# Pixie8888/R3DFSSeg

Hardware: AMD Instinct MI355X
Metric: episodes/sec S3DIS 2-way 5-shot 2048-pt (MPTI+attention, train step: forward+backward+grad all-reduce+Adam) (higher is better)
Workload: dtype f32 (index-free GEMMs -- self-attention, 1x1 convolutions, weight gradients, the EdgeConv backward's edge GEMMs -- as bf16x3 split products on the bf16 MFMA with fp32 accumulate; every index-deciding result: fp32)

## Files before the change

### r3dfsseg_amd/csrc/edge_tile.h

```cpp
#pragma once
#include "common.h"

#define E2_PTS 4
#define E2_LD 68

static __device__ __forceinline__ f32x4 mfma16(float a, float b, f32x4 c) {
  return __builtin_amdgcn_mfma_f32_16x16x4f32(a, b, c, 0, 0, 0);
}

template <int RT>
static __device__ __forceinline__ void e2_rowgemm(const float* __restrict__ A, const float (&Bf)[16], int n, int g,
                                                  f32x4 (&acc)[RT]) {
#pragma unroll
  for (int t = 0; t < RT; ++t) acc[t] = f32x4{0.f, 0.f, 0.f, 0.f};
#pragma unroll
  for (int qk = 0; qk < 4; ++qk) {
    float4 av[RT];
#pragma unroll
    for (int t = 0; t < RT; ++t) av[t] = *(const float4*)(A + (16 * t + n) * E2_LD + 16 * g + 4 * qk);
#pragma unroll
    for (int s = 0; s < 4; ++s) {
#pragma unroll
      for (int t = 0; t < RT; ++t) {
        const float a = s == 0 ? av[t].x : s == 1 ? av[t].y : s == 2 ? av[t].z : av[t].w;
        acc[t] = mfma16(a, Bf[4 * qk + s], acc[t]);
      }
    }
  }
}

template <typename KernelT>
static int e2_resident_blocks(KernelT kernel, size_t lds, int cap) {
  if (hipFuncSetAttribute((const void*)kernel, hipFuncAttributeMaxDynamicSharedMemorySize, (int)lds) != hipSuccess) return 0;
  int per_cu = 0, dev = 0;
  hipDeviceProp_t prop;
  if (hipOccupancyMaxActiveBlocksPerMultiprocessor(&per_cu, kernel, 256, lds) != hipSuccess || hipGetDevice(&dev) != hipSuccess ||
      hipGetDeviceProperties(&prop, dev) != hipSuccess || per_cu <= 0)
    return 0;
  const int r = per_cu * prop.multiProcessorCount;
  return r < cap ? r : cap;
// ... 2 lines not shown
```

### r3dfsseg_amd/csrc/edgeconv.hip

```cpp
#include "edge_tile.h"

template <int RT>
__global__ __launch_bounds__(256) void r3d_edgeconv_kernel(
    const float* __restrict__ PQ, const int* __restrict__ idx, const float* __restrict__ W2,
    const float* __restrict__ s2, const float* __restrict__ t2, float* __restrict__ out, long ldo,
    int N, long total_points, int* __restrict__ argmax_out) {
  constexpr int K = 4 * RT, R = 16 * RT;
  extern __shared__ __attribute__((aligned(16))) float smem[];
  float* H = smem;
  float* Z = smem + R * E2_LD;
  const int tid = threadIdx.x, lane = tid & 63, w = tid >> 6;
  const int n = lane & 15, g = lane >> 4;
  const int c = 16 * w + n;
  float Bz[16];
#pragma unroll
  for (int s = 0; s < 16; ++s) Bz[s] = W2[c * 64 + 16 * g + s];
  const float s2c = s2[c], t2c = t2[c];
  const long units = total_points / E2_PTS;
  for (long item = blockIdx.x; item < units; item += gridDim.x) {
    const long u = r3d_xcd_swizzle((int)item, (int)units);
    const long pt0 = u * E2_PTS;
    const long cloud0 = (pt0 / N) * N;
    {
      const int my_idx = min(max(idx[(pt0 + w) * K + min(lane, K - 1)], 0), N - 1);
      const float q = PQ[(pt0 + w) * 128 + 64 + lane];
      float pv[K];
#pragma unroll
      for (int t = 0; t < K; ++t) pv[t] = PQ[(cloud0 + __builtin_amdgcn_readlane(my_idx, t)) * 128 + lane];
      float* hrow = H + (K * w) * E2_LD + lane;
#pragma unroll
      for (int t = 0; t < K; ++t) {
        const float h = pv[t] + q;
        hrow[t * E2_LD] = h > 0.f ? h : 0.2f * h;
      }
    }
    __syncthreads();
    f32x4 acc[RT];
    e2_rowgemm<RT>(H, Bz, n, g, acc);
#pragma unroll
    for (int t = 0; t < RT; ++t) {
#pragma unroll
      for (int i = 0; i < 4; ++i) {
        const float v = s2c * acc[t][i] + t2c;
        Z[(16 * t + 4 * g + i) * E2_LD + c] = v > 0.f ? v : 0.2f * v;
      }
    }
    __syncthreads();
    {
      const float* zp = Z + (K * w) * E2_LD + lane;
      float m = zp[0];
      int am = 0;
#pragma unroll
      for (int t = 1; t < K; ++t) {
        const float v = zp[t * E2_LD];
        if (v > m) { m = v; am = t; }
      }
      out[(pt0 + w) * ldo + lane] = m;
      if (argmax_out) argmax_out[(pt0 + w) * 64 + lane] = am;
    }
  }
}

template <int RT>
static int edgeconv_launch_rt(const float* PQ, const int32_t* idx, const float* W2, const float* s2, const float* t2, float* out,
                              long ldo, int N, long total_points, int32_t* argmax_out, hipStream_t st) {
  const size_t lds = sizeof(float) * ((size_t)2 * 16 * RT * E2_LD);
  static int resident = 0;
  if (!resident) {
    resident = e2_resident_blocks(r3d_edgeconv_kernel<RT>, lds, 1024);
    R3D_REQUIRE(resident > 0, "r3d_edgeconv_fwd: cannot reserve %zu B of LDS", lds);
  }
  const long units = total_points / E2_PTS;
  const int grid = (int)(units <= resident ? units : (resident & ~7));
  hipLaunchKernelGGL(r3d_edgeconv_kernel<RT>, dim3(grid), dim3(256), lds, st, PQ, idx, W2, s2, t2, out, ldo, N, total_points,
                     argmax_out);
  return R3D_OK;
}

extern "C" int r3d_edgeconv_fwd(const float* PQ, const int32_t* idx, const float* W2, const float* s2,
                                const float* t2, float* out, long ldo, int B, int N, int K,
                                int32_t* argmax_out, void* stream) {
  R3D_REQUIRE(PQ && idx && W2 && s2 && t2 && out, "r3d_edgeconv_fwd: null pointer");
  R3D_REQUIRE(B > 0 && N > 0 && ldo >= 64, "r3d_edgeconv_fwd: bad shape");
  R3D_REQUIRE(N % E2_PTS == 0, "r3d_edgeconv_fwd: N=%d must be a multiple of %d", N, E2_PTS);
  R3D_REQUIRE(K >= 4 && K <= 32 && K % 4 == 0, "r3d_edgeconv_fwd: K=%d unsupported (need K %% 4 == 0, 4..32)", K);
  hipStream_t st = (hipStream_t)stream;
  int rc = R3D_ERR_ARG;
#define E2_CASE(RT) \
  case RT: rc = edgeconv_launch_rt<RT>(PQ, idx, W2, s2, t2, out, ldo, N, (long)B * N, argmax_out, st); break
  switch (K / 4) {
    E2_CASE(1); E2_CASE(2); E2_CASE(3); E2_CASE(4); E2_CASE(5); E2_CASE(6); E2_CASE(7); E2_CASE(8);
  }
#undef E2_CASE
  if (rc) return rc;
  R3D_LAUNCH_CHECK("r3d_edgeconv_fwd");
  return R3D_OK;
}
```

### r3dfsseg_amd/csrc/edgeconv_train.hip

```cpp
#include <stdlib.h>
#include "edge_tile.h"

#define ET_LD 65
#define ET_MAXBLK 1024
#define EC_CHUNK 32

static __device__ __forceinline__ float lrelu(float v) { return v > 0.f ? v : 0.2f * v; }

struct EcGeom {
  int N, cpc;
  __host__ __device__ static EcGeom make(int N) { return EcGeom{N, (N + EC_CHUNK - 1) / EC_CHUNK}; }
  __device__ void range(int chunk, int& cloud, int& p0, int& p1) const {
    cloud = __builtin_amdgcn_readfirstlane(chunk / cpc);
    p0 = __builtin_amdgcn_readfirstlane(cloud * N + (chunk - cloud * cpc) * EC_CHUNK);
    p1 = __builtin_amdgcn_readfirstlane(min(p0 + EC_CHUNK, (cloud + 1) * N));
  }
};
static __device__ __forceinline__ int ec_seg(const r3d_segmap& cs, int cloud) {
  return __builtin_amdgcn_readfirstlane(cs.seg_of_row32(cloud));
}

template <int RT>
__global__ __launch_bounds__(256) void r3d_edge_stats1_kernel(const float* __restrict__ PQ, const int* __restrict__ idx,
                                                              EcGeom gm, int n_chunks, float* __restrict__ part,
// ... 200 lines not shown
        float bs = 0.f, es = 0.f;
#pragma unroll
        for (int t = 0; t < K; ++t) {
          const float v = grow[t * E2_LD];
          drow[t * 64] = v;
          bs += v;
          es += eh[t];
          sdye += v * eh[t];
        }
        sdy += bs;
        BE[(pt0 + w) * 128 + lane] = bs;
        BE[(pt0 + w) * 128 + 64 + lane] = es;
      }
    }
    float (*ps)[2][64] = (float (*)[2][64])dsm;
    ps[w][0][lane] = sdy;
    ps[w][1][lane] = sdye;
    __syncthreads();
    if (tid < 128) {
      const int v = tid >> 6, cc = tid & 63;
      part_bn[((long)chunk * 2 + v) * 64 + cc] = ((ps[0][v][cc] + ps[1][v][cc]) + ps[2][v][cc]) + ps[3][v][cc];
    }
    __syncthreads();
  }
  int tid2 = threadIdx.x;
  asm volatile("" : "+v"(tid2));
  const int w2 = tid2 >> 6, n2 = tid2 & 15, g2 = (tid2 >> 4) & 3;
  float* mypart = part_dw + (long)blockIdx.x * 4096;
#pragma unroll
  for (int i = 0; i < 4; ++i)
    *(float4*)(mypart + (16 * w2 + 4 * g2 + i) * 64 + 4 * n2) = float4{dw[0][i], dw[1][i], dw[2][i], dw[3][i]};
}

template <int RT>
__global__ __launch_bounds__(256) void r3d_edgeconv_train_fwd2_kernel(
    const float* __restrict__ PQ, const int* __restrict__ idx, const float* __restrict__ s1, const float* __restrict__ t1,
    long bn_stride, const float* __restrict__ W2, EcGeom gm, r3d_segmap cs , int n_chunks,
    int* __restrict__ argmax_out, float* __restrict__ zmax_out, float* __restrict__ zmin_out, int* __restrict__ argmin_out,
    float* __restrict__ part ) {
  constexpr int K = 4 * RT, R = 16 * RT;
  extern __shared__ __attribute__((aligned(16))) float smem[];
  float* H = smem;
  float* Z = smem + R * E2_LD;
  const int tid = threadIdx.x, lane = tid & 63, w = tid >> 6;
  const int n = lane & 15, g = lane >> 4;
  const int c = 16 * w + n;
  const int N = gm.N;
  float Bz[16];
#pragma unroll
  for (int s = 0; s < 16; ++s) Bz[s] = W2[c * 64 + 16 * g + s];
  for (int item = blockIdx.x; item < n_chunks; item += gridDim.x) {
    const int chunk = r3d_xcd_swizzle(item, n_chunks);
    int cloud, p0, p1;
    gm.range(chunk, cloud, p0, p1);
    const long cloud0 = (long)cloud * N;
    const long bo = (long)ec_seg(cs, cloud) * bn_stride;
    const float sc1 = s1[bo + lane], sh1 = t1[bo + lane];
    float za = 0.f, zb = 0.f;
    for (int pt0_ = p0; pt0_ < p1; pt0_ += E2_PTS) {
      const long pt0 = pt0_;
      {
        const int my_idx = min(max(idx[(pt0 + w) * K + min(lane, K - 1)], 0), N - 1);
        const float q = PQ[(pt0 + w) * 128 + 64 + lane];
        float pv[K];
#pragma unroll
        for (int t = 0; t < K; ++t) pv[t] = PQ[(cloud0 + __builtin_amdgcn_readlane(my_idx, t)) * 128 + lane];
        float* hrow = H + (K * w) * E2_LD + lane;
#pragma unroll
        for (int t = 0; t < K; ++t) hrow[t * E2_LD] = lrelu(sc1 * (pv[t] + q) + sh1);
      }
      __syncthreads();
      f32x4 acc[RT];
      e2_rowgemm<RT>(H, Bz, n, g, acc);
#pragma unroll
      for (int t = 0; t < RT; ++t) {
#pragma unroll
        for (int i = 0; i < 4; ++i) {
          const float z = acc[t][i];
          za += z;
          zb += z * z;
          Z[(16 * t + 4 * g + i) * E2_LD + c] = z;
        }
      }
      __syncthreads();
      {
        const float* zp = Z + (K * w) * E2_LD + lane;
        float zx = zp[0], zn = zx;
        int ax = 0, an = 0;
#pragma unroll
        for (int t = 1; t < K; ++t) {
          const float z = zp[t * E2_LD];
          if (z > zx) { zx = z; ax = t; }
          if (z < zn) { zn = z; an = t; }
        }
        const long o = (pt0 + w) * 64 + lane;
        zmax_out[o] = zx;
        zmin_out[o] = zn;
        argmax_out[o] = ax;
        argmin_out[o] = an;
      }
    }
    za += __shfl_xor(za, 16); zb += __shfl_xor(zb, 16);
    za += __shfl_xor(za, 32); zb += __shfl_xor(zb, 32);
    if (g == 0) {
      part[((long)chunk * 2 + 0) * 64 + c] = za;
      part[((long)chunk * 2 + 1) * 64 + c] = zb;
    }
  }
}

#define RV_RANGE 256
#define RV_CAP 12288
__global__ __launch_bounds__(1024) void r3d_edge_reverse_kernel(const int* __restrict__ idx, int N, int K, int n_clouds,
                                                                int* __restrict__ rev_ptr, int* __restrict__ rev) {
  __shared__ int cnt[RV_RANGE];
  __shared__ int off[RV_RANGE + 1];
  __shared__ int cur[RV_RANGE];
  __shared__ int buf[RV_CAP];
  __shared__ int wsum[16];
  __shared__ int below_s, b_s;
  const int tid = threadIdx.x, lane = tid & 63, w = tid >> 6;
  const int cloud = blockIdx.y;
  const int r0 = blockIdx.x * RV_RANGE, nr = min(RV_RANGE, N - r0);
  const long E = (long)N * K, gbase = (long)cloud * E;
  const int* lst = idx + gbase;
  if (tid < RV_RANGE) cnt[tid] = 0;
  if (tid == 0) below_s = 0;
  __syncthreads();
  int my_below = 0;
  for (long e0 = tid; e0 < E; e0 += 8 * 1024) {
    int jv[8];
#pragma unroll
    for (int u = 0; u < 8; ++u) jv[u] = lst[min(e0 + 1024 * u, E - 1)];
// ... 239 lines not shown

extern "C" long r3d_edgeconv_train_ws_words(int B, int N) { return (long)ET_MAXBLK * 4096 + (long)et_chunks(B, N) * 128 + 64; }

static void et_reduce_chunks(const float* part, int N, int clouds_a, int clouds_b, int n_seg, float* out, hipStream_t st) {
  const int cpc = EcGeom::make(N).cpc;
  hipLaunchKernelGGL(r3d_part_reduce_kernel, dim3(128 / 64, n_seg), dim3(1024), 0, st, part, clouds_a * cpc, clouds_b * cpc, 128,
                     out, 128L, 128, (float*)nullptr, 0L);
}

extern "C" int r3d_edge_stats1(const float* PQ, const int32_t* idx, int B, int N, int K, int clouds_a, int clouds_b,
                               float* sums_out, float* esum, float* ws, void* stream) {
  R3D_REQUIRE(PQ && idx && sums_out && ws, "r3d_edge_stats1: null pointer");
  int rc = et_check("r3d_edge_stats1", B, N, K, clouds_a, clouds_b);
  if (rc) return rc;
  hipStream_t st = (hipStream_t)stream;
  const EcGeom gm = EcGeom::make(N);
  const int n_chunks = et_chunks(B, N);
  const int grid = et_grid8(n_chunks, 2048);
#define E2_CASE(RT) \
  case RT: hipLaunchKernelGGL(r3d_edge_stats1_kernel<RT>, dim3(grid), dim3(256), 0, st, PQ, idx, gm, n_chunks, ws, esum); break
  switch (K / 4) {
    E2_CASE(1); E2_CASE(2); E2_CASE(3); E2_CASE(4); E2_CASE(5); E2_CASE(6); E2_CASE(7); E2_CASE(8);
  }
#undef E2_CASE
  et_reduce_chunks(ws, N, clouds_a, clouds_b, r3d_segmap{clouds_a, clouds_b}.n_seg(B), sums_out, st);
  R3D_LAUNCH_CHECK("r3d_edge_stats1");
  return R3D_OK;
}

template <int RT>
static int fwd2_launch_rt(int n_chunks, hipStream_t st, const float* PQ, const int32_t* idx, const float* s1, const float* t1,
                          long bn_stride, const float* W2, EcGeom gm, r3d_segmap cs, int32_t* argmax, float* zmax, float* zmin,
                          int32_t* argmin, float* ws) {
  const size_t lds = sizeof(float) * ((size_t)2 * 16 * RT * E2_LD);
  static int resident = 0;
  if (!resident) {
    resident = e2_resident_blocks(r3d_edgeconv_train_fwd2_kernel<RT>, lds, ET_MAXBLK);
    R3D_REQUIRE(resident > 0, "r3d_edgeconv_train_fwd_minmax: cannot reserve %zu B of LDS", lds);
  }
  const int grid = et_grid8(n_chunks, resident);
  hipLaunchKernelGGL(r3d_edgeconv_train_fwd2_kernel<RT>, dim3(grid), dim3(256), lds, st, PQ, idx, s1, t1, bn_stride, W2, gm, cs,
                     n_chunks, argmax, zmax, zmin, argmin, ws);
  return R3D_OK;
}

extern "C" int r3d_edgeconv_train_fwd_minmax(const float* PQ, const int32_t* idx, const float* s1, const float* t1,
                                             long bn_stride, const float* W2, int B, int N, int K, int clouds_a, int clouds_b,
                                             float* zmax, float* zmin, int32_t* argmax, int32_t* argmin, float* sums_out,
                                             float* ws, void* stream) {
  R3D_REQUIRE(PQ && idx && s1 && t1 && W2 && zmax && zmin && argmax && argmin && sums_out && ws,
              "r3d_edgeconv_train_fwd_minmax: null pointer");
  int rc = et_check("r3d_edgeconv_train_fwd_minmax", B, N, K, clouds_a, clouds_b);
  if (rc) return rc;
  hipStream_t st = (hipStream_t)stream;
  const EcGeom gm = EcGeom::make(N);
  const r3d_segmap cs{clouds_a, clouds_b};
  const int n_chunks = et_chunks(B, N);
#define E2_CASE(RT)                                                                                                    \
  case RT:                                                                                                             \
    rc = fwd2_launch_rt<RT>(n_chunks, st, PQ, idx, s1, t1, bn_stride, W2, gm, cs, argmax, zmax, zmin, argmin, ws);      \
    break
  switch (K / 4) {
    E2_CASE(1); E2_CASE(2); E2_CASE(3); E2_CASE(4); E2_CASE(5); E2_CASE(6); E2_CASE(7); E2_CASE(8);
  }
#undef E2_CASE
  if (rc) return rc;
  et_reduce_chunks(ws, N, clouds_a, clouds_b, cs.n_seg(B), sums_out, st);
// ... 149 lines not shown
```

### r3dfsseg_amd/csrc/knn.hip

```cpp
#include <stdlib.h>
#include "common.h"

#define KNN_Q 32
#define KNN_CH 128
#define KNN_SLAB 64
#define KNN_ROWS_PER_WAVE 8


__global__ void r3d_sqnorm_kernel(const float* __restrict__ x, long ldx, int rows, int C,
                                  float* __restrict__ out) {
  int i = blockIdx.x * blockDim.x + threadIdx.x;
  if (i >= rows) return;
  const float* p = x + (long)i * ldx;
  float acc = 0.f;
  for (int c = 0; c < C; ++c) acc = __builtin_fmaf(p[c], p[c], acc);
  out[i] = acc;
}

template <int R>
struct TopList {
  float v[R];
  int id[R];
};

// ... 519 lines not shown
  const int b = lin / (int)gridDim.x, tile_x = lin - b * (int)gridDim.x;
  const int n = n_dev ? min(n_dev[(long)b * n_dev_stride], N) : N;
  const int q0 = tile_x * 32;
  if (q0 >= n) return;
  const int tid = threadIdx.x, lane = tid & 63, w = tid >> 6;
  const int h = lane >> 5, j = lane & 31;
  const int nch = (C + 2 * KCH - 1) / (2 * KCH);
  const int Cs = nch * 2 * KCH + (BFB ? 4 : 1);
  float* Aq = smem;
  float* region = smem + 32 * Cs;
  const float* xb = xT + (long)b * C * ldT;
  const float* nb = nrm + (long)b * N;

  for (int e = tid; e < 32 * nch * 2 * KCH; e += 64 * KB_WAVES) {
    const int c = e >> 5, jj = e & 31;
    const float v = xb[(long)min(c, C - 1) * ldT + min(q0 + jj, n - 1)];
    Aq[jj * Cs + c] = r3d_keep(v, c < C && q0 + jj < n);
  }
  if (tid < 32) cnt_s[tid] = 0;
  const int Cp = nch * 64;
  const int QRS = 2 * Cp + 8;
  unsigned short* Aqb = reinterpret_cast<unsigned short*>(region + ((32 * (KB_TOP * KB_GROUPS + 1) + 3) & ~3));
  const unsigned short* xpb = BFA ? xpk + (long)b * N * 2 * Cp : nullptr;
  if (BFA) {
    const int cpr = 2 * Cp / 8;
    for (int e = tid; e < 32 * cpr; e += 64 * KB_WAVES) {
      const int c8 = e >> 5, jj = e & 31;
      *reinterpret_cast<r3d_u32x4*>(Aqb + jj * QRS + 8 * c8) =
          *reinterpret_cast<const r3d_u32x4*>(xpb + ((long)c8 * N + min(q0 + jj, n - 1)) * 8);
    }
  }
  KSTAMP(8);
  float nq[16];
#pragma unroll
  for (int r = 0; r < 16; ++r) {
    const int row = q0 + r3d_acc_row(r, lane);
    nq[r] = r3d_keep(nb[min(row, n - 1)], row < n);
  }
  const float* cnb = BFA ? cnorm + (long)b * N : nullptr;
  const float slack = (float)(C + 8) * 0x1p-24f;
  auto bound_k = [&](int i) { return cnb[i] * (1.f + 0x1p-12f) + nb[i] * slack; };
  float* kq_s = reinterpret_cast<float*>(Aqb + 32 * QRS);
  if (BFA && tid < 32) kq_s[tid] = bound_k(min(q0 + tid, n - 1));
  auto bound_ku = [&](int i) { return cnb[i] * (1.f - 0x1p-12f) - nb[i] * slack; };
  if (BFB && tid < 32) kq_s[32 + tid] = bound_ku(min(q0 + tid, n - 1));
  __syncthreads();

  const int nsub = ((n + 31) / 32 - z + nsplit - 1) / nsplit;
  const int my_sub = (nsub - w + KB_WAVES - 1) / KB_WAVES;
  const int T = (w < nsub) ? my_sub * nch : 0;

  int stride = KB_SAMPLE;
  auto bload = [&](int t, float (&bf)[KCH]) {
    const int st = (w + KB_WAVES * stride * (t / nch)) * nsplit + z, ch = (t % nch);
    const int cand = 32 * st + j;
    const bool ok = cand < n;
    const int cc = min(cand, n - 1);
    if (FULLC) {
      const float* p = xb + (long)(2 * KCH * ch + h) * ldT + cc;
      const long st2 = 2 * ldT;
#pragma unroll
      for (int s = 0; s < KCH; ++s) bf[s] = p[s * st2];
    } else {
#pragma unroll
      for (int s = 0; s < KCH; ++s) {
        const int c = 2 * KCH * ch + 2 * s + h;
        bf[s] = r3d_keep(xb[(long)min(c, C - 1) * ldT + cc], ok && c < C);
      }
    }
  };
  f32x16 acc;
  auto mma = [&](int t, const float (&bf)[KCH]) {
    const int ch = (t % nch);
    if (ch == 0) {
#pragma unroll
      for (int r = 0; r < 16; ++r) acc[r] = 0.f;
    }
    const float* ap = Aq + j * Cs + 2 * KCH * ch + h;
    float av[KCH];
#pragma unroll
    for (int s = 0; s < KCH; ++s) av[s] = ap[2 * s];
    __builtin_amdgcn_sched_barrier(0);
#pragma unroll
    for (int s = 0; s < KCH; ++s) acc = __builtin_amdgcn_mfma_f32_32x32x2f32(av[s], bf[s], acc, 0, 0, 0);
  };
  float kb[16];
  auto load_kb = [&](int which) {
#pragma unroll
    for (int r = 0; r < 16; ++r) kb[r] = kq_s[32 * which + r3d_acc_row(r, lane)];
  };
  auto scores_lb = [&](int st, f32x16& sc) {
    const int cand = 32 * st + j;
    const float kj = bound_k(min(cand, n - 1));
#pragma unroll
    for (int r = 0; r < 16; ++r) {
      const float v = __builtin_fmaf(2.f, acc[r], -(kb[r] + kj));
      sc[r] = SMODE == R3D_SCORE_DGCNN ? v : fminf(v, 0.f);
    }
    if (32 * st + 32 > n) {
      const bool valid = cand < n;
#pragma unroll
      for (int r = 0; r < 16; ++r) sc[r] = valid ? sc[r] : -INFINITY;
    }
  };
  auto scores_ub = [&](int st, f32x16& sc) {
    const int cand = 32 * st + j;
    const float kj = bound_ku(min(cand, n - 1));
#pragma unroll
    for (int r = 0; r < 16; ++r) {
      const float v = __builtin_fmaf(2.f, acc[r], -(kb[r] + kj));
      sc[r] = SMODE == R3D_SCORE_DGCNN ? v : fminf(v, 0.f);
    }
    if (32 * st + 32 > n) {
      const bool valid = cand < n;
#pragma unroll
      for (int r = 0; r < 16; ++r) sc[r] = valid ? sc[r] : -INFINITY;
    }
  };
  auto scores = [&](int st, f32x16& sc) {
    const int cand = 32 * st + j;
    const bool valid = cand < n;
    const float nj = r3d_keep(nb[min(cand, n - 1)], valid);
#pragma unroll
    for (int r = 0; r < 16; ++r) {
      float v;
      if (SMODE == R3D_SCORE_DGCNN) {
        const float inner = -2.f * acc[r];
        v = ((-nj) - inner) - nq[r];
      } else {
        const float dis = (nq[r] + nj) - 2.f * acc[r];
        v = -fmaxf(dis, 0.f);
      }
      sc[r] = v;
    }
    if (32 * st + 32 > n) {
#pragma unroll
      for (int r = 0; r < 16; ++r) sc[r] = valid ? sc[r] : -INFINITY;
    }
  };

  float bfA[KCH], bfB[KCH];
  float g1[16], g2[16];
#pragma unroll
  for (int r = 0; r < 16; ++r) { g1[r] = -INFINITY; g2[r] = -INFINITY; }
  auto finishA_sub = [&](int i) {
    f32x16 sc;
    if (BFA) scores_lb((w + KB_WAVES * stride * i) * nsplit + z, sc);
    else scores((w + KB_WAVES * stride * i) * nsplit + z, sc);
#pragma unroll
    for (int r = 0; r < 16; ++r) {
      const float x = sc[r];
      if (KB_TOP == 2) {
        const float lo = fminf(g1[r], x);
        g2[r] = fmaxf(g2[r], lo);
      }
      g1[r] = fmaxf(g1[r], x);
    }
  };
  auto finishA = [&](int t) {
    if ((t % nch) == nch - 1) finishA_sub(t / nch);
  };
  KSTAMP(9);
  const int TA = (w < nsub) ? ((my_sub + KB_SAMPLE - 1) / KB_SAMPLE) * nch : 0;
  r3d_u32x4 pfA[8], pfB[8];
  const __amdgpu_buffer_rsrc_t rpk = __builtin_amdgcn_make_buffer_rsrc(
      (void*)(BFA ? xpb : (const unsigned short*)xT), 0, BFA ? (int)((long)N * 2 * Cp * 2) : 0, 0x00020000);
  const int chunk_b = N * 16;
  auto pload = [&](int i, int ch, r3d_u32x4 (&pf)[8]) {
    const int st = (w + KB_WAVES * stride * i) * nsplit + z;
    const int cc = min(32 * st + j, n - 1);
    const int voff = (h * N + cc) * 16;
    const int soff = 8 * ch * chunk_b, lo = (Cp / 8) * chunk_b;
#pragma unroll
    for (int s4 = 0; s4 < 4; ++s4) {
      pf[2 * s4] = __builtin_amdgcn_raw_buffer_load_b128(rpk, voff, soff + 2 * s4 * chunk_b, 0);
      pf[2 * s4 + 1] = __builtin_amdgcn_raw_buffer_load_b128(rpk, voff, soff + lo + 2 * s4 * chunk_b, 0);
    }
  };
  auto pmma = [&](int ch, const r3d_u32x4 (&pf)[8]) {
    if (ch == 0) {
#pragma unroll
      for (int r = 0; r < 16; ++r) acc[r] = 0.f;
    }
    const unsigned short* ap = Aqb + j * QRS + 64 * ch + 8 * h;
#pragma unroll
    for (int half = 0; half < 2; ++half) {
      r3d_u32x4 ah[2], al[2];
#pragma unroll
      for (int u = 0; u < 2; ++u) {
        ah[u] = *reinterpret_cast<const r3d_u32x4*>(ap + 16 * (2 * half + u));
        al[u] = *reinterpret_cast<const r3d_u32x4*>(ap + Cp + 16 * (2 * half + u));
      }
#pragma unroll
      for (int u = 0; u < 2; ++u) {
        const int s4 = 2 * half + u;
        acc = r3d_mfma_bf16(al[u], pf[2 * s4], acc);
// ... 2 lines not shown
      }
    }
  };
  auto bf_pass = [&](int n_sub, auto&& finish) {
    const int U = n_sub * nch;
    if (U <= 0) return;
    int i_c = 0, ch_c = 0, i_n = 0, ch_n = 0;
    auto advance = [&](int& i, int& ch) {
      if (++ch == nch) { ch = 0; ++i; }
    };
    pload(0, 0, pfA);
    advance(i_n, ch_n);
    int u = 0;
    for (; u + 1 < U; u += 2) {
      pload(i_n, ch_n, pfB);
      __builtin_amdgcn_sched_barrier(0);
      pmma(ch_c, pfA);
      if (ch_c == nch - 1) finish(i_c);
      i_c = i_n; ch_c = ch_n;
      advance(i_n, ch_n);
      const bool more = u + 2 < U;
      pload(more ? i_n : i_c, more ? ch_n : ch_c, pfA);
      __builtin_amdgcn_sched_barrier(0);
      pmma(ch_c, pfB);
      if (ch_c == nch - 1) finish(i_c);
      i_c = i_n; ch_c = ch_n;
      advance(i_n, ch_n);
    }
    if (u < U) {
      pmma(ch_c, pfA);
      if (ch_c == nch - 1) finish(i_c);
    }
  };
  if (BFA) {
    load_kb(0);
    bf_pass((w < nsub) ? (my_sub + KB_SAMPLE - 1) / KB_SAMPLE : 0, finishA_sub);
  } else {
    if (TA > 0) bload(0, bfB);
    for (int t = 0; t < TA; ++t) {
#pragma unroll
      for (int s = 0; s < KCH; ++s) bfA[s] = bfB[s];
      if (t + 1 < TA) bload(t + 1, bfB);
      __builtin_amdgcn_sched_barrier(0);
      mma(t, bfA);
      finishA(t);
    }
  }
  KSTAMP(10);
  stride = 1;
  {
    constexpr int GS = KB_TOP * KB_GROUPS + 1;
#pragma unroll
    for (int r = 0; r < 16; ++r) {
      const int q = r3d_acc_row(r, lane);
      region[q * GS + KB_TOP * (32 * w + j)] = g1[r];
      if (KB_TOP == 2) region[q * GS + 2 * (32 * w + j) + 1] = g2[r];
    }
    __syncthreads();
    for (int qq = 0; qq < 32 / KB_WAVES; ++qq) {
      const int q = (32 / KB_WAVES) * w + qq;
      unsigned key[KB_TOP * KB_GROUPS / 64];
#pragma unroll
      for (int i = 0; i < KB_TOP * KB_GROUPS / 64; ++i) key[i] = f2key(region[q * GS + 64 * i + lane]) >> 16;
      unsigned res = 0;
      for (int bit = 15; bit >= 0; --bit) {
        const unsigned cand = res | (1u << bit);
        int c = 0;
#pragma unroll
        for (int i = 0; i < KB_TOP * KB_GROUPS / 64; ++i) c += __popcll(__ballot(key[i] >= cand));
        if (c >= k) res = cand;
      }
      if (lane == 0) tau_s[q] = key2f(res << 16);
    }
    __syncthreads();
  }
  KSTAMP(11);
  float tauq[16];
#pragma unroll
  for (int r = 0; r < 16; ++r) tauq[r] = q0 + r3d_acc_row(r, lane) < n ? tau_s[r3d_acc_row(r, lane)] : INFINITY;
  __syncthreads();

  static_assert(!BFB || 32 * KB_CAP <= 32 * (KB_TOP * KB_GROUPS + 1), "the index buffer must end in front of the query pieces");
  float* bufv = region + (BFB ? 32 * KB_CAP : 0);
  int* bufi = (int*)(region + (BFB ? 0 : 32 * KB_CAP));
  constexpr bool BMP = BFB && KB_WAVES == 4;
  unsigned* bm = reinterpret_cast<unsigned*>(region);
  bool overflow = false;
  auto finishB = [&](int t) {
    if ((t % nch) != nch - 1) return;
    const int st = (w + KB_WAVES * (t / nch)) * nsplit + z;
    f32x16 sc;
    scores(st, sc);
#pragma unroll
    for (int r = 0; r < 16; ++r) {
      if (sc[r] >= tauq[r]) {
        const int q = r3d_acc_row(r, lane);
        const int slot = atomicAdd(&cnt_s[q], 1);
        if (slot < KB_CAP) {
          bufv[q * KB_CAP + slot] = sc[r];
          bufi[q * KB_CAP + slot] = 32 * st + j;
        } else {
          overflow = true;
        }
      }
    }
  };
  auto finishBF = [&](int i) {
    const int st = (w + KB_WAVES * i) * nsplit + z;
    f32x16 sc;
    scores_ub(st, sc);
    if (BMP) {
      unsigned long long m[16];
#pragma unroll
      for (int r = 0; r < 16; ++r) m[r] = __ballot(sc[r] >= tauq[r]);
      __builtin_amdgcn_sched_barrier(0);
      int word = 0;
#define KB_LO(r) "s"((int)(unsigned)(m[r] & 0xffffffffull))
#define KB_HI(r) "s"((int)(unsigned)(m[r] >> 32))
      asm volatile(
                   "s_nop 4\n\t"
                   "v_writelane_b32 %0, %1, 0\n\t"
                   "v_writelane_b32 %0, %2, 4\n\t"
                   "v_writelane_b32 %0, %3, 1\n\t"
                   "v_writelane_b32 %0, %4, 5\n\t"
                   "v_writelane_b32 %0, %5, 2\n\t"
                   "v_writelane_b32 %0, %6, 6\n\t"
                   "v_writelane_b32 %0, %7, 3\n\t"
                   "v_writelane_b32 %0, %8, 7\n\t"
                   "v_writelane_b32 %0, %9, 8\n\t"
// ... 17 lines not shown
                   "v_writelane_b32 %0, %7, 19\n\t"
                   "v_writelane_b32 %0, %8, 23\n\t"
                   "v_writelane_b32 %0, %9, 24\n\t"
                   "v_writelane_b32 %0, %10, 28\n\t"
                   "v_writelane_b32 %0, %11, 25\n\t"
                   "v_writelane_b32 %0, %12, 29\n\t"
                   "v_writelane_b32 %0, %13, 26\n\t"
                   "v_writelane_b32 %0, %14, 30\n\t"
                   "v_writelane_b32 %0, %15, 27\n\t"
                   "v_writelane_b32 %0, %16, 31"
                   : "+v"(word)
                   : KB_LO(8), KB_HI(8), KB_LO(9), KB_HI(9), KB_LO(10), KB_HI(10), KB_LO(11), KB_HI(11), KB_LO(12), KB_HI(12), KB_LO(13), KB_HI(13), KB_LO(14), KB_HI(14), KB_LO(15), KB_HI(15));
#undef KB_LO
#undef KB_HI
      __builtin_amdgcn_sched_barrier(0);
      const int ls = w + KB_WAVES * i;
      if (lane < 32) bm[ls * 32 + ((lane + ls) & 31)] = (unsigned)word;
      return;
    }
#pragma unroll
    for (int r = 0; r < 16; ++r) {
      if (sc[r] >= tauq[r]) {
        const int q = r3d_acc_row(r, lane);
        const int slot = atomicAdd(&cnt_s[q], 1);
        if (slot < KB_CAP) bufi[q * KB_CAP + slot] = 32 * st + j;
        else overflow = true;
      }
    }
  };
  if (BFB) {
    load_kb(1);
    bf_pass((w < nsub) ? my_sub : 0, finishBF);
  } else {
    if (T > 0) bload(0, bfB);
    for (int t = 0; t < T; ++t) {
#pragma unroll
      for (int s = 0; s < KCH; ++s) bfA[s] = bfB[s];
      if (t + 1 < T) bload(t + 1, bfB);
      __builtin_amdgcn_sched_barrier(0);
      mma(t, bfA);
      finishB(t);
    }
  }
  KSTAMP(12);
  if (BMP) {
    __syncthreads();
    constexpr int QW = 32 / KB_WAVES, NCH = (KB_CAP + 63) / 64;
    unsigned wq[QW][NCH];
#pragma unroll
    for (int i = 0; i < QW; ++i)
#pragma unroll
      for (int cch = 0; cch < NCH; ++cch) {
        const int ls = 64 * cch + lane;
        wq[i][cch] = ls < nsub ? bm[ls * 32 + ((QW * w + i + ls) & 31)] : 0u;
      }
    __syncthreads();
#pragma unroll
    for (int i = 0; i < QW; ++i) {
      const int q = QW * w + i;
      int total = 0;
#pragma unroll
      for (int cch = 0; cch < NCH; ++cch) {
        if (64 * cch >= nsub) break;
        unsigned word = wq[i][cch];
        const int c = __popc(word);
        const int incl = r3d_wave_incl_scan(c);
        int off = total + incl - c;
        const int cand0 = 32 * ((64 * cch + lane) * nsplit + z);
        while (word) {
          const int bit = __ffs((int)word) - 1;
          if (off < KB_CAP) bufi[q * KB_CAP + off] = cand0 + bit;
          ++off;
          word &= word - 1;
        }
        total += __builtin_amdgcn_readlane(incl, 63);
// ... 499 lines not shown
  const KnnChoice ch = knn_choose(p, g_knn_bf16_threshold, g_knn_bf16_filter, x, (int)(ldx & 3), ((uintptr_t)x & 15) == 0);
  KnnCall c = {x, ldx, nullptr, 0, B, N, C, k, mode, n_valid_dev, n_valid_stride, idx_out, score_out, (hipStream_t)stream};
  if (ws) {
    R3D_REQUIRE(((uintptr_t)ws & 15) == 0 && ws_words >= p.words,
                "r3d_knn_topk_batched: ws must be 16-byte aligned and hold r3d_knn_ws_words = %ld floats (got %ld)", p.words,
                ws_words);
    c.norms = ws + p.norms;
    c.tile_flags = (int*)(ws + p.tile_flags);
    c.cm = ws + p.xcm;
    c.pieces = (unsigned short*)(ws + p.pieces);
    c.mean = ws + p.mean;
    c.cnorm = ws + p.cnorm;
    c.split_idx = (int*)(ws + p.split_idx);
    c.split_sc = ws + p.split_sc;
  } else {
    c.norms = norm_ws;
    c.tile_flags = (int*)(norm_ws + (long)B * N);
    c.cm = cm_ws;
  }
  if (ch.path == KNN_INSERTION) {
    R3D_REQUIRE(c.x, "r3d_knn_topk: the insertion kernel needs the point-major matrix");
    const size_t lds = knn_lds_bytes(c.C);
    R3D_REQUIRE(lds <= 160 * 1024, "r3d_knn_topk: C=%d needs %zu B of LDS (> 160 KiB)", c.C, lds);
    int rc = knn_sqnorm_launch(c.x, c.ldx, (long)c.B * c.N, c.C, c.norms, c.st);
    if (rc) return rc;
    if (ch.regs == 1) knn_insertion_launch<1>(c, lds);
    else if (ch.regs == 2) knn_insertion_launch<2>(c, lds);
    else knn_insertion_launch<4>(c, lds);
    R3D_LAUNCH_CHECK("r3d_knn_topk");
    return R3D_OK;
  }
  int rc = knn_cm_operand(c, x_cm);
  if (rc) return rc;
  const dim3 grid(r3d_cdiv(c.N, 32), c.B);
  if (ch.path == KNN_STREAMED_SMALL) {
    r3d_zero_words(c.tile_flags, (long)c.B * grid.x, c.st);
    if (ch.chan == R3D_KNN_CHAN_LE16) {
      rc = ch.few ? knn_append_launch<8, KM_CAP, KM_TOP, 8, KM_SAMPLE, false>(c, grid, nullptr, c.tile_flags)
                 : knn_append_launch<KM_WAVES, KM_CAP, KM_TOP, 8, KM_SAMPLE, false>(c, grid, nullptr, c.tile_flags);
    } else if (ch.bfa) {
      knn_pack_bf(c);
      rc = ch.filter ? knn_append_launch<KM_WAVES, KM_CAP, KM_TOP, 32, 1, true, true, true>(c, grid, nullptr, c.tile_flags)
                     : knn_append_launch<KM_WAVES, KM_CAP, KM_TOP, 32, KM_SAMPLE, true, true>(c, grid, nullptr, c.tile_flags);
    } else if (ch.chan == R3D_KNN_CHAN_FULL) {
      rc = ch.few ? knn_append_launch<8, KM_CAP, KM_TOP, 32, KM_SAMPLE, true>(c, grid, nullptr, c.tile_flags)
                 : knn_append_launch<KM_WAVES, KM_CAP, KM_TOP, 32, KM_SAMPLE, true>(c, grid, nullptr, c.tile_flags);
    } else {
      rc = ch.few ? knn_append_launch<8, KM_CAP, KM_TOP, 32, KM_SAMPLE, false>(c, grid, nullptr, c.tile_flags)
                 : knn_append_launch<KM_WAVES, KM_CAP, KM_TOP, 32, KM_SAMPLE, false>(c, grid, nullptr, c.tile_flags);
    }
    if (rc) return rc;
    hipLaunchKernelGGL(ch.chan == R3D_KNN_CHAN_LE16 ? r3d_knn_small_kernel<8> : r3d_knn_small_kernel<32>, grid, dim3(256), 0, c.st,
                       c.xT, c.ldT, c.N, c.C, c.k, c.mode, c.n_dev, c.n_stride, c.norms, c.idx, c.sc, (const int*)c.tile_flags);
    R3D_LAUNCH_CHECK("r3d_knn_topk(small)");
    return R3D_OK;
  }
  r3d_zero_words(status, 1, c.st);
  const dim3 gb(grid.x, c.B, ch.split ? 2 : 1);
  if (ch.bfa) {
    knn_pack_bf(c);
    rc = knn_append_launch<8, 384, 2, 32, 1, true, true>(c, gb, status, nullptr);
  } else if (ch.chan == R3D_KNN_CHAN_FULL) {
    rc = knn_append_launch<8, 384, 2, 32, 1, true>(c, gb, status, nullptr);
  } else {
    rc = knn_append_launch<8, 384, 2, 32, 1, false>(c, gb, status, nullptr);
  }
// ... 23 lines not shown
```

Before: 404.9.

## Reorder EdgeConv H rows so max-pool happens in MFMA registers, drop Z LDS

Permutes the row layout of the edge-feature tile H so that each lane's MFMA accumulator holds all K neighbours of a single (point, channel) pair. The max/min pooling, argmax/argmin and BN statistics can then be computed directly from registers, with no Z scratch buffer in LDS and no second read pass. LDS per block is halved, which may allow more resident blocks. The output stores now use a (point = g, channel = c) lane mapping, which changes how stores coalesce.

```diff
diff --git a/r3dfsseg_amd/csrc/edge_tile.h b/r3dfsseg_amd/csrc/edge_tile.h
--- a/r3dfsseg_amd/csrc/edge_tile.h
+++ b/r3dfsseg_amd/csrc/edge_tile.h
@@ -6,6 +6,21 @@
 
 static __device__ __forceinline__ f32x4 mfma16(float a, float b, f32x4 c) {
   return __builtin_amdgcn_mfma_f32_16x16x4f32(a, b, c, 0, 0, 0);
+}
+
+static __device__ __forceinline__ int e2_hrow(int p, int e) { return 16 * (e >> 2) + 4 * p + (e & 3); }
+
+template <int K>
+static __device__ __forceinline__ int e2_list(const int* __restrict__ idx, long pt, int N, int lane) {
+  return min(max(idx[pt * K + min(lane, K - 1)], 0), N - 1);
+}
+
+template <int K>
+static __device__ __forceinline__ void e2_gather(const float* __restrict__ PQ, long cloud0, long pt, int my_idx, int lane,
+                                                 float& q, float (&pv)[K]) {
+  q = PQ[pt * 128 + 64 + lane];
+#pragma unroll
+  for (int t = 0; t < K; ++t) pv[t] = PQ[(cloud0 + __builtin_amdgcn_readlane(my_idx, t)) * 128 + lane];
 }
 
 template <int RT>
diff --git a/r3dfsseg_amd/csrc/edgeconv.hip b/r3dfsseg_amd/csrc/edgeconv.hip
--- a/r3dfsseg_amd/csrc/edgeconv.hip
+++ b/r3dfsseg_amd/csrc/edgeconv.hip
@@ -1,14 +1,31 @@
 #include "edge_tile.h"
+
+template <int RT>
+static __device__ __forceinline__ void e2_pool_store(const f32x4 (&acc)[RT], float s2c, float t2c, float* __restrict__ out,
+                                                     int* __restrict__ am_out) {
+  float m = 0.f;
+  int am = 0;
+#pragma unroll
+  for (int t = 0; t < RT; ++t) {
+#pragma unroll
+    for (int i = 0; i < 4; ++i) {
+      float v = s2c * acc[t][i] + t2c;
+      v = v > 0.f ? v : 0.2f * v;
+      if (t + i == 0) m = v;
+      else if (v > m) { m = v; am = 4 * t + i; }
+    }
+  }
+  *out = m;
+  if (am_out) *am_out = am;
+}
 
 template <int RT>
 __global__ __launch_bounds__(256) void r3d_edgeconv_kernel(
     const float* __restrict__ PQ, const int* __restrict__ idx, const float* __restrict__ W2,
     const float* __restrict__ s2, const float* __restrict__ t2, float* __restrict__ out, long ldo,
     int N, long total_points, int* __restrict__ argmax_out) {
-  constexpr int K = 4 * RT, R = 16 * RT;
-  extern __shared__ __attribute__((aligned(16))) float smem[];
-  float* H = smem;
-  float* Z = smem + R * E2_LD;
+  constexpr int K = 4 * RT;
+  extern __shared__ __attribute__((aligned(16))) float H[];
   const int tid = threadIdx.x, lane = tid & 63, w = tid >> 6;
   const int n = lane & 15, g = lane >> 4;
   const int c = 16 * w + n;
@@ -22,49 +39,27 @@
     const long pt0 = u * E2_PTS;
     const long cloud0 = (pt0 / N) * N;
     {
-      const int my_idx = min(max(idx[(pt0 + w) * K + min(lane, K - 1)], 0), N - 1);
-      const float q = PQ[(pt0 + w) * 128 + 64 + lane];
-      float pv[K];
-#pragma unroll
-      for (int t = 0; t < K; ++t) pv[t] = PQ[(cloud0 + __builtin_amdgcn_readlane(my_idx, t)) * 128 + lane];
-      float* hrow = H + (K * w) * E2_LD + lane;
+      const int my_idx = e2_list<K>(idx, pt0 + w, N, lane);
+      float q, pv[K];
+      e2_gather<K>(PQ, cloud0, pt0 + w, my_idx, lane, q, pv);
 #pragma unroll
       for (int t = 0; t < K; ++t) {
         const float h = pv[t] + q;
-        hrow[t * E2_LD] = h > 0.f ? h : 0.2f * h;
+        H[e2_hrow(w, t) * E2_LD + lane] = h > 0.f ? h : 0.2f * h;
       }
     }
     __syncthreads();
     f32x4 acc[RT];
     e2_rowgemm<RT>(H, Bz, n, g, acc);
-#pragma unroll
-    for (int t = 0; t < RT; ++t) {
-#pragma unroll
-      for (int i = 0; i < 4; ++i) {
-        const float v = s2c * acc[t][i] + t2c;
-        Z[(16 * t + 4 * g + i) * E2_LD + c] = v > 0.f ? v : 0.2f * v;
-      }
-    }
     __syncthreads();
-    {
-      const float* zp = Z + (K * w) * E2_LD + lane;
-      float m = zp[0];
-      int am = 0;
-#pragma unroll
-      for (int t = 1; t < K; ++t) {
-        const float v = zp[t * E2_LD];
-        if (v > m) { m = v; am = t; }
-      }
-      out[(pt0 + w) * ldo + lane] = m;
-      if (argmax_out) argmax_out[(pt0 + w) * 64 + lane] = am;
-    }
+    e2_pool_store<RT>(acc, s2c, t2c, out + (pt0 + g) * ldo + c, argmax_out ? argmax_out + (pt0 + g) * 64 + c : nullptr);
   }
 }
 
 template <int RT>
 static int edgeconv_launch_rt(const float* PQ, const int32_t* idx, const float* W2, const float* s2, const float* t2, float* out,
                               long ldo, int N, long total_points, int32_t* argmax_out, hipStream_t st) {
-  const size_t lds = sizeof(float) * ((size_t)2 * 16 * RT * E2_LD);
+  const size_t lds = sizeof(float) * ((size_t)16 * RT * E2_LD);
   static int resident = 0;
   if (!resident) {
     resident = e2_resident_blocks(r3d_edgeconv_kernel<RT>, lds, 1024);
diff --git a/r3dfsseg_amd/csrc/edgeconv_train.hip b/r3dfsseg_amd/csrc/edgeconv_train.hip
--- a/r3dfsseg_amd/csrc/edgeconv_train.hip
+++ b/r3dfsseg_amd/csrc/edgeconv_train.hip
@@ -256,16 +256,39 @@
     *(float4*)(mypart + (16 * w2 + 4 * g2 + i) * 64 + 4 * n2) = float4{dw[0][i], dw[1][i], dw[2][i], dw[3][i]};
 }
 
+
+template <int RT>
+static __device__ __forceinline__ void et_pool_store(const f32x4 (&acc)[RT], float& za, float& zb, long o,
+                                                     float* __restrict__ zmax_out, float* __restrict__ zmin_out,
+                                                     int* __restrict__ argmax_out, int* __restrict__ argmin_out) {
+  float zx = acc[0][0], zn = zx;
+  int ax = 0, an = 0;
+#pragma unroll
+  for (int t = 0; t < RT; ++t) {
+#pragma unroll
+    for (int i = 0; i < 4; ++i) {
+      const float z = acc[t][i];
+      za += z;
+      zb += z * z;
+      if (z > zx) { zx = z; ax = 4 * t + i; }
+      if (z < zn) { zn = z; an = 4 * t + i; }
+    }
+  }
+  zmax_out[o] = zx;
+  zmin_out[o] = zn;
+  argmax_out[o] = ax;
+  argmin_out[o] = an;
+}
+
 template <int RT>
 __global__ __launch_bounds__(256) void r3d_edgeconv_train_fwd2_kernel(
     const float* __restrict__ PQ, const int* __restrict__ idx, const float* __restrict__ s1, const float* __restrict__ t1,
     long bn_stride, const float* __restrict__ W2, EcGeom gm, r3d_segmap cs , int n_chunks,
     int* __restrict__ argmax_out, float* __restrict__ zmax_out, float* __restrict__ zmin_out, int* __restrict__ argmin_out,
     float* __restrict__ part ) {
-  constexpr int K = 4 * RT, R = 16 * RT;
+  constexpr int K = 4 * RT;
   extern __shared__ __attribute__((aligned(16))) float smem[];
   float* H = smem;
-  float* Z = smem + R * E2_LD;
   const int tid = threadIdx.x, lane = tid & 63, w = tid >> 6;
   const int n = lane & 15, g = lane >> 4;
   const int c = 16 * w + n;
@@ -284,45 +307,17 @@
     for (int pt0_ = p0; pt0_ < p1; pt0_ += E2_PTS) {
       const long pt0 = pt0_;
       {
-        const int my_idx = min(max(idx[(pt0 + w) * K + min(lane, K - 1)], 0), N - 1);
-        const float q = PQ[(pt0 + w) * 128 + 64 + lane];
-        float pv[K];
-#pragma unroll
-        for (int t = 0; t < K; ++t) pv[t] = PQ[(cloud0 + __builtin_amdgcn_readlane(my_idx, t)) * 128 + lane];
-        float* hrow = H + (K * w) * E2_LD + lane;
-#pragma unroll
-        for (int t = 0; t < K; ++t) hrow[t * E2_LD] = lrelu(sc1 * (pv[t] + q) + sh1);
+        const int my_idx = e2_list<K>(idx, pt0 + w, N, lane);
+        float q, pv[K];
+        e2_gather<K>(PQ, cloud0, pt0 + w, my_idx, lane, q, pv);
+#pragma unroll
+        for (int t = 0; t < K; ++t) H[e2_hrow(w, t) * E2_LD + lane] = lrelu(sc1 * (pv[t] + q) + sh1);
       }
       __syncthreads();
       f32x4 acc[RT];
       e2_rowgemm<RT>(H, Bz, n, g, acc);
-#pragma unroll
-      for (int t = 0; t < RT; ++t) {
-#pragma unroll
-        for (int i = 0; i < 4; ++i) {
-          const float z = acc[t][i];
-          za += z;
-          zb += z * z;
-          Z[(16 * t + 4 * g + i) * E2_LD + c] = z;
-        }
-      }
       __syncthreads();
-      {
-        const float* zp = Z + (K * w) * E2_LD + lane;
-        float zx = zp[0], zn = zx;
-        int ax = 0, an = 0;
-#pragma unroll
-        for (int t = 1; t < K; ++t) {
-          const float z = zp[t * E2_LD];
-          if (z > zx) { zx = z; ax = t; }
-          if (z < zn) { zn = z; an = t; }
-        }
-        const long o = (pt0 + w) * 64 + lane;
-        zmax_out[o] = zx;
-        zmin_out[o] = zn;
-        argmax_out[o] = ax;
-        argmin_out[o] = an;
-      }
+      et_pool_store<RT>(acc, za, zb, (pt0 + g) * 64 + c, zmax_out, zmin_out, argmax_out, argmin_out);
     }
     za += __shfl_xor(za, 16); zb += __shfl_xor(zb, 16);
     za += __shfl_xor(za, 32); zb += __shfl_xor(zb, 32);
@@ -628,7 +623,7 @@
 static int fwd2_launch_rt(int n_chunks, hipStream_t st, const float* PQ, const int32_t* idx, const float* s1, const float* t1,
                           long bn_stride, const float* W2, EcGeom gm, r3d_segmap cs, int32_t* argmax, float* zmax, float* zmin,
                           int32_t* argmin, float* ws) {
-  const size_t lds = sizeof(float) * ((size_t)2 * 16 * RT * E2_LD);
+  const size_t lds = sizeof(float) * ((size_t)16 * RT * E2_LD);
   static int resident = 0;
   if (!resident) {
     resident = e2_resident_blocks(r3d_edgeconv_train_fwd2_kernel<RT>, lds, ET_MAXBLK);
```

Measured after the change: 406.2, median of 4. About the same (+0.3%).

## Pipeline fp32 KNN candidate loads via buffer loads with double-buffered fragments

Applied to the files above, without the earlier changes.

Replaces the fp32 (non-BFA) candidate streaming loop in the KNN append kernel with a double-buffered pass that uses raw buffer loads for the candidate columns and their norms. The candidate norm is prefetched alongside the fragment instead of being reloaded in the scoring step. For the single-chunk case the query operand is hoisted into registers once. The query-norm load is deferred on the BFA path to reduce register pressure. This is meant to hide global-load latency behind MFMA work. In exchange it adds register pressure and a 2 GiB buffer-size limit check.

```diff
diff --git a/r3dfsseg_amd/csrc/knn.hip b/r3dfsseg_amd/csrc/knn.hip
--- a/r3dfsseg_amd/csrc/knn.hip
+++ b/r3dfsseg_amd/csrc/knn.hip
@@ -575,11 +575,14 @@
   }
   KSTAMP(8);
   float nq[16];
-#pragma unroll
-  for (int r = 0; r < 16; ++r) {
-    const int row = q0 + r3d_acc_row(r, lane);
-    nq[r] = r3d_keep(nb[min(row, n - 1)], row < n);
-  }
+  auto load_nq = [&]() {
+#pragma unroll
+    for (int r = 0; r < 16; ++r) {
+      const int row = q0 + r3d_acc_row(r, lane);
+      nq[r] = r3d_keep(nb[min(row, n - 1)], row < n);
+    }
+  };
+  if (!BFA) load_nq();
   const float* cnb = BFA ? cnorm + (long)b * N : nullptr;
   const float slack = (float)(C + 8) * 0x1p-24f;
   auto bound_k = [&](int i) { return cnb[i] * (1.f + 0x1p-12f) + nb[i] * slack; };
@@ -591,41 +594,55 @@
 
   const int nsub = ((n + 31) / 32 - z + nsplit - 1) / nsplit;
   const int my_sub = (nsub - w + KB_WAVES - 1) / KB_WAVES;
-  const int T = (w < nsub) ? my_sub * nch : 0;
 
   int stride = KB_SAMPLE;
-  auto bload = [&](int t, float (&bf)[KCH]) {
-    const int st = (w + KB_WAVES * stride * (t / nch)) * nsplit + z, ch = (t % nch);
-    const int cand = 32 * st + j;
-    const bool ok = cand < n;
-    const int cc = min(cand, n - 1);
-    if (FULLC) {
-      const float* p = xb + (long)(2 * KCH * ch + h) * ldT + cc;
-      const long st2 = 2 * ldT;
-#pragma unroll
-      for (int s = 0; s < KCH; ++s) bf[s] = p[s * st2];
+  const __amdgpu_buffer_rsrc_t rx = __builtin_amdgcn_make_buffer_rsrc((void*)xb, 0, (int)((long)C * ldT * 4), 0x00020000);
+  const __amdgpu_buffer_rsrc_t rn = __builtin_amdgcn_make_buffer_rsrc((void*)nb, 0, N * 4, 0x00020000);
+  const int ld_b = (int)ldT * 4;
+  const int half_b = h ? ld_b : 0;
+  struct F32Frag {
+    float bf[KCH];
+    float nj;
+  };
+  const int w_s = __builtin_amdgcn_readfirstlane(w);
+  auto fload = [&](int sub_stride, int i, int ch, F32Frag& f) {
+    const int st = (w_s + KB_WAVES * sub_stride * i) * nsplit + z;
+    const int cc = min(32 * st + j, n - 1);
+    const int voff = half_b + 4 * cc + (KCH == 8 ? 0 : ch * (2 * KCH * ld_b));
+#pragma unroll
+    for (int s = 0; s < KCH; ++s)
+      f.bf[s] = __int_as_float(__builtin_amdgcn_raw_buffer_load_b32(rx, voff, 2 * s * ld_b, 0));
+    f.nj = __int_as_float(__builtin_amdgcn_raw_buffer_load_b32(rn, 4 * cc, 0, 0));
+  };
+  f32x16 acc;
+  constexpr bool ONE_CHUNK = KCH == 8;
+  float qv[ONE_CHUNK ? KCH : 1];
+  if (ONE_CHUNK) {
+#pragma unroll
+    for (int s = 0; s < KCH; ++s) qv[s] = Aq[j * Cs + h + 2 * s];
+  }
+  auto fmma = [&](int ch, const F32Frag& f) {
+    if (ONE_CHUNK || ch == 0) {
+#pragma unroll
+      for (int r = 0; r < 16; ++r) acc[r] = 0.f;
+    }
+    if (ONE_CHUNK) {
+#pragma unroll
+      for (int s = 0; s < KCH; ++s) acc = __builtin_amdgcn_mfma_f32_32x32x2f32(qv[s], f.bf[s], acc, 0, 0, 0);
     } else {
-#pragma unroll
-      for (int s = 0; s < KCH; ++s) {
-        const int c = 2 * KCH * ch + 2 * s + h;
-        bf[s] = r3d_keep(xb[(long)min(c, C - 1) * ldT + cc], ok && c < C);
-      }
-    }
-  };
-  f32x16 acc;
-  auto mma = [&](int t, const float (&bf)[KCH]) {
-    const int ch = (t % nch);
-    if (ch == 0) {
-#pragma unroll
-      for (int r = 0; r < 16; ++r) acc[r] = 0.f;
-    }
-    const float* ap = Aq + j * Cs + 2 * KCH * ch + h;
-    float av[KCH];
-#pragma unroll
-    for (int s = 0; s < KCH; ++s) av[s] = ap[2 * s];
-    __builtin_amdgcn_sched_barrier(0);
-#pragma unroll
-    for (int s = 0; s < KCH; ++s) acc = __builtin_amdgcn_mfma_f32_32x32x2f32(av[s], bf[s], acc, 0, 0, 0);
+      const float* ap = Aq + j * Cs + 2 * KCH * ch + h;
+      constexpr int AV = (KB_WAVES == 4 && FULLC) ? KCH / 2 : KCH;
+#pragma unroll
+      for (int s0 = 0; s0 < KCH; s0 += AV) {
+        float av[AV];
+#pragma unroll
+        for (int s = 0; s < AV; ++s) av[s] = ap[2 * (s0 + s)];
+        __builtin_amdgcn_sched_barrier(0);
+#pragma unroll
+        for (int s = 0; s < AV; ++s) acc = __builtin_amdgcn_mfma_f32_32x32x2f32(av[s], f.bf[s0 + s], acc, 0, 0, 0);
+        if (AV < KCH) __builtin_amdgcn_sched_barrier(0);
+      }
+    }
   };
   float kb[16];
   auto load_kb = [&](int which) {
@@ -660,10 +677,10 @@
       for (int r = 0; r < 16; ++r) sc[r] = valid ? sc[r] : -INFINITY;
     }
   };
-  auto scores = [&](int st, f32x16& sc) {
+  auto scores = [&](int st, float nj_cc , f32x16& sc) {
     const int cand = 32 * st + j;
     const bool valid = cand < n;
-    const float nj = r3d_keep(nb[min(cand, n - 1)], valid);
+    const float nj = r3d_keep(nj_cc, valid);
 #pragma unroll
     for (int r = 0; r < 16; ++r) {
       float v;
@@ -682,14 +699,14 @@
     }
   };
 
-  float bfA[KCH], bfB[KCH];
+  F32Frag bfA, bfB;
   float g1[16], g2[16];
 #pragma unroll
   for (int r = 0; r < 16; ++r) { g1[r] = -INFINITY; g2[r] = -INFINITY; }
-  auto finishA_sub = [&](int i) {
+  auto finishA_sub = [&](int i, float nj = 0.f) {
     f32x16 sc;
     if (BFA) scores_lb((w + KB_WAVES * stride * i) * nsplit + z, sc);
-    else scores((w + KB_WAVES * stride * i) * nsplit + z, sc);
+    else scores((w + KB_WAVES * stride * i) * nsplit + z, nj, sc);
 #pragma unroll
     for (int r = 0; r < 16; ++r) {
       const float x = sc[r];
@@ -700,11 +717,7 @@
       g1[r] = fmaxf(g1[r], x);
     }
   };
-  auto finishA = [&](int t) {
-    if ((t % nch) == nch - 1) finishA_sub(t / nch);
-  };
   KSTAMP(9);
-  const int TA = (w < nsub) ? ((my_sub + KB_SAMPLE - 1) / KB_SAMPLE) * nch : 0;
   r3d_u32x4 pfA[8], pfB[8];
   const __amdgpu_buffer_rsrc_t rpk = __builtin_amdgcn_make_buffer_rsrc(
       (void*)(BFA ? xpb : (const unsigned short*)xT), 0, BFA ? (int)((long)N * 2 * Cp * 2) : 0, 0x00020000);
@@ -773,19 +786,43 @@
       if (ch_c == nch - 1) finish(i_c);
     }
   };
+  auto f32_pass = [&](int n_sub, int sub_stride, auto&& finish) {
+    const int U = __builtin_amdgcn_readfirstlane(n_sub) * (ONE_CHUNK ? 1 : nch);
+    if (U <= 0) return;
+    int i_c = 0, ch_c = 0, i_n = 0, ch_n = 0;
+    auto advance = [&](int& i, int& ch) {
+      if (ONE_CHUNK) { ++i; return; }
+      if (++ch == nch) { ch = 0; ++i; }
+    };
+    auto last = [&](int ch) { return ONE_CHUNK || ch == nch - 1; };
+    fload(sub_stride, 0, 0, bfA);
+    advance(i_n, ch_n);
+    int u = 0;
+    for (; u + 1 < U; u += 2) {
+      fload(sub_stride, i_n, ch_n, bfB);
+      __builtin_amdgcn_sched_barrier(0);
+      fmma(ch_c, bfA);
+      if (last(ch_c)) finish(i_c, bfA.nj);
+      i_c = i_n; ch_c = ch_n;
+      advance(i_n, ch_n);
+      const bool more = u + 2 < U;
+      fload(sub_stride, more ? i_n : i_c, more ? ch_n : ch_c, bfA);
+      __builtin_amdgcn_sched_barrier(0);
+      fmma(ch_c, bfB);
+      if (last(ch_c)) finish(i_c, bfB.nj);
+      i_c = i_n; ch_c = ch_n;
+      advance(i_n, ch_n);
+    }
+    if (u < U) {
+      fmma(ch_c, bfA);
+      if (last(ch_c)) finish(i_c, bfA.nj);
+    }
+  };
   if (BFA) {
     load_kb(0);
     bf_pass((w < nsub) ? (my_sub + KB_SAMPLE - 1) / KB_SAMPLE : 0, finishA_sub);
   } else {
-    if (TA > 0) bload(0, bfB);
-    for (int t = 0; t < TA; ++t) {
-#pragma unroll
-      for (int s = 0; s < KCH; ++s) bfA[s] = bfB[s];
-      if (t + 1 < TA) bload(t + 1, bfB);
-      __builtin_amdgcn_sched_barrier(0);
-      mma(t, bfA);
-      finishA(t);
-    }
+    f32_pass((w < nsub) ? (my_sub + KB_SAMPLE - 1) / KB_SAMPLE : 0, stride, finishA_sub);
   }
   KSTAMP(10);
   stride = 1;
@@ -816,6 +853,7 @@
     __syncthreads();
   }
   KSTAMP(11);
+  if (BFA) load_nq();
   float tauq[16];
 #pragma unroll
   for (int r = 0; r < 16; ++r) tauq[r] = q0 + r3d_acc_row(r, lane) < n ? tau_s[r3d_acc_row(r, lane)] : INFINITY;
@@ -827,15 +865,17 @@
   constexpr bool BMP = BFB && KB_WAVES == 4;
   unsigned* bm = reinterpret_cast<unsigned*>(region);
   bool overflow = false;
-  auto finishB = [&](int t) {
-    if ((t % nch) != nch - 1) return;
-    const int st = (w + KB_WAVES * (t / nch)) * nsplit + z;
+  auto finishB = [&](int i, float nj) {
+    const int st = (w + KB_WAVES * i) * nsplit + z;
     f32x16 sc;
-    scores(st, sc);
+    scores(st, nj, sc);
+    constexpr bool TIGHT = KB_WAVES == 4 && FULLC && KCH == 32;
 #pragma unroll
     for (int r = 0; r < 16; ++r) {
       if (sc[r] >= tauq[r]) {
-        const int q = r3d_acc_row(r, lane);
+        int lane_q = lane;
+        if (TIGHT) asm volatile("" : "+v"(lane_q));
+        const int q = r3d_acc_row(r, lane_q);
         const int slot = atomicAdd(&cnt_s[q], 1);
         if (slot < KB_CAP) {
           bufv[q * KB_CAP + slot] = sc[r];
@@ -919,15 +959,7 @@
     load_kb(1);
     bf_pass((w < nsub) ? my_sub : 0, finishBF);
   } else {
-    if (T > 0) bload(0, bfB);
-    for (int t = 0; t < T; ++t) {
-#pragma unroll
-      for (int s = 0; s < KCH; ++s) bfA[s] = bfB[s];
-      if (t + 1 < T) bload(t + 1, bfB);
-      __builtin_amdgcn_sched_barrier(0);
-      mma(t, bfA);
-      finishB(t);
-    }
+    f32_pass((w < nsub) ? my_sub : 0, 1, finishB);
   }
   KSTAMP(12);
   if (BMP) {
@@ -1493,6 +1525,7 @@
   }
   int rc = knn_cm_operand(c, x_cm);
   if (rc) return rc;
+  R3D_REQUIRE((long)c.C * c.ldT * 4 <= 0x7fffffffL, "r3d_knn_topk: a point set of C=%d x pitch %ld floats exceeds 2 GiB", c.C, c.ldT);
   const dim3 grid(r3d_cdiv(c.N, 32), c.B);
   if (ch.path == KNN_STREAMED_SMALL) {
     r3d_zero_words(c.tile_flags, (long)c.B * grid.x, c.st);
```

New measurement: 405.3 before, 411.6 after, median of 6. 1.5% higher.
